# Gyeeta/gyeeta

Hardware: NVIDIA H100
Metric: events/sec aggregated (higher is better)
Workload: dtype u64

## Files before the change

gyeeta_b200/csrc/gysk_tdigest.cuh:

```cuda
#pragma once

#include "gysk_device.cuh"

namespace gysk {

struct TdParams { const double *qtab; uint32_t delta; uint32_t pad; };

template <int NMAX_>
struct TdWorkT
{
	static constexpr int NMAX = NMAX_;
	double			mean[NMAX];
	unsigned long long	pref[NMAX + 1];
	uint16_t		bounds[TD_CAP + 2];
	uint16_t		nxt[NMAX];
	double			src[NMAX];
};
using TdWork = TdWorkT<2 * TD_CAP>;
using TdWorkBig = TdWorkT<1120>;
struct TdScratch : TdWork
{
	Centroid		newc[TD_CAP];
};

template <bool B_STAGED, typename Work>
__device__ __forceinline__ uint32_t td_merge_compress(Work &S, const Centroid *a, uint32_t na, const Centroid *b, uint32_t nb,
		Centroid *out, const TdParams &P)
{
	const int lane = threadIdx.x & 31;
	const uint32_t nm = na + nb;

	double *am = S.src, *bm = S.src + na;
	for (uint32_t j0 = 0; j0 < na; j0 += 32 * 4) {
		double v[4];
#pragma unroll
		for (int q = 0; q < 4; ++q) { const uint32_t j = j0 + q * 32 + lane; v[q] = j < na ? a[j].mean : 0.0; }
#pragma unroll
		for (int q = 0; q < 4; ++q) { const uint32_t j = j0 + q * 32 + lane; if (j < na) am[j] = v[q]; }
	}
	if (!B_STAGED) for (uint32_t j = lane; j < nb; j += 32) bm[j] = b[j].mean;
	__syncwarp();
	const uint32_t per = (nm + 31u) >> 5;
	const uint32_t d0 = lane * per < nm ? lane * per : nm, d1 = d0 + per < nm ? d0 + per : nm;
	unsigned long long tot = 0;
	if (d0 < d1) {
		uint32_t lo = d0 > nb ? d0 - nb : 0u, hi = d0 < na ? d0 : na;
		while (lo < hi) { const uint32_t mid = (lo + hi) >> 1; if (am[mid] <= bm[d0 - 1u - mid]) lo = mid + 1; else hi = mid; }
		uint32_t i = lo, k = d0 - lo;
		double av = i < na ? am[i] : 0.0, bv = k < nb ? bm[k] : 0.0;
		constexpr unsigned long long FROM_A = 1ull << 63;
		for (uint32_t pos = d0; pos < d1; ++pos) {
			const bool ta = i < na && (k >= nb || av <= bv);
			S.mean[pos] = ta ? av : bv;
			if (B_STAGED) S.pref[pos + 1] = ta ? (FROM_A | i) : (unsigned long long)S.nxt[k];
			else S.nxt[pos] = (uint16_t)(ta ? i : (0x8000u | k));
			if (ta) { ++i; av = i < na ? am[i] : 0.0; }
			else { ++k; bv = k < nb ? bm[k] : 0.0; }
		}
		for (uint32_t p0 = d0; p0 < d1; p0 += 4) {
			unsigned long long w[4];
#pragma unroll
			for (int q = 0; q < 4; ++q) {
				const uint32_t pos = p0 + q < d1 ? p0 + q : d1 - 1u;
				if (B_STAGED) { const unsigned long long f = S.pref[pos + 1]; w[q] = (f & FROM_A) ? a[(uint32_t)f].weight : f; }
				else { const uint32_t from = S.nxt[pos]; w[q] = (from & 0x8000u) ? b[from & 0x7FFFu].weight : a[from].weight; }
			}
#pragma unroll
			for (int q = 0; q < 4; ++q) if (p0 + q < d1) { S.pref[p0 + q + 1] = w[q]; tot += w[q]; }
		}
	}
	{
		unsigned long long incl = tot;
#pragma unroll
		for (int off = 1; off < 32; off <<= 1) {
			const unsigned long long tt = __shfl_up_sync(0xffffffffu, incl, off);
			if (lane >= off) incl += tt;
		}
		unsigned long long run = incl - tot;
		for (uint32_t pos = d0; pos < d1; ++pos) { run += S.pref[pos + 1]; S.pref[pos + 1] = run; }
		if (lane == 0) S.pref[0] = 0;
	}
	__syncwarp();
	auto ckey = [&S](uint32_t i) { const unsigned long long p = S.pref[i]; return p + ((S.pref[i + 1] - p) >> 1); };

	uint32_t nout = 0;
	if (nm) {
		const unsigned long long Wt = S.pref[nm];
		const double W = (double)Wt;
		const uint32_t cj = (P.delta + 32u) >> 5;
		uint32_t lo = 0;
		for (uint32_t j = lane * cj, jn = 0; jn < cj && j <= P.delta; ++j, ++jn) {
			const unsigned long long T = j == P.delta ? Wt : (unsigned long long)__dmul_rn(__ldg(P.qtab + j), W);
			uint32_t steps = jn ? 0u : 8u;
			while (steps < 8u && lo < nm && ckey(lo) < T) { ++lo; ++steps; }
			if (steps == 8u) {
				uint32_t hi = nm;
				while (lo < hi) { const uint32_t mid = (lo + hi) >> 1; if (ckey(mid) < T) lo = mid + 1; else hi = mid; }
			}
			S.nxt[j] = (uint16_t)lo;
		}
		__syncwarp();
		for (uint32_t j0 = 0; j0 < P.delta; j0 += 32) {
			const uint32_t j = j0 + lane;
			const bool ne = j < P.delta && S.nxt[j + 1] > S.nxt[j];
			const uint32_t m = __ballot_sync(0xffffffffu, ne);
			if (ne) S.bounds[nout + __popc(m & ((1u << lane) - 1u))] = S.nxt[j];
			nout += __popc(m);
		}
		if (lane == 0) S.bounds[nout] = (uint16_t)nm;
		__syncwarp();
	}

	for (uint32_t c = lane; c < nout; c += 32) {
		double csum = 0.0;
		const uint32_t lo = S.bounds[c], hi = S.bounds[c + 1];
		for (uint32_t i = lo; i < hi; ++i) {
			csum = __dadd_rn(csum, __dmul_rn(S.mean[i], (double)(S.pref[i + 1] - S.pref[i])));
		}
		const unsigned long long cw = S.pref[hi] - S.pref[lo];
		Centroid o; o.mean = __ddiv_rn(csum, (double)cw); o.weight = cw;
		out[c] = o;
	}
	__syncwarp();
	return nout;
}

template <typename Work>
__device__ __forceinline__ uint32_t warp_merge_compress(Work &S, const Centroid *a, uint32_t na, const Centroid *b, uint32_t nb,
		Centroid *out, const TdParams &P)
{
	return td_merge_compress<false>(S, a, na, b, nb, out, P);
}

template <typename Work>
__device__ __forceinline__ uint32_t warp_merge_compress_staged(Work &S, const Centroid *a, uint32_t na, uint32_t nb, Centroid *out,
		const TdParams &P)
{
	return td_merge_compress<true>(S, a, na, nullptr, nb, out, P);
}

}
```

Measured before the change: 13.46 billion.

## Invert t-digest cell lookup per centroid via arcsine estimate and register-cached weights

Instead of binary-searching each of the delta quantile thresholds against the centroid cumulative keys, each merged centroid now estimates its cell index from the arcsine scale function in float and corrects it with a short local walk over a threshold table held in shared scratch. Cell boundaries come from comparing neighbouring cell indices with shuffles and ballots. Input A's weights are also loaded together with the means into registers and staged in shared memory, so the weight gather no longer does scattered global reads. This depends on the float estimate landing close to the right cell, keeps more registers live (sized by TD_CAP), and adds warp syncs.

```diff
diff --git a/gyeeta_b200/csrc/gysk_tdigest.cuh b/gyeeta_b200/csrc/gysk_tdigest.cuh
--- a/gyeeta_b200/csrc/gysk_tdigest.cuh
+++ b/gyeeta_b200/csrc/gysk_tdigest.cuh
@@ -10,6 +10,7 @@
 struct TdWorkT
 {
 	static constexpr int NMAX = NMAX_;
+	static_assert(NMAX > TD_CAP, "the compress keeps the cell starts T_0 .. T_delta (delta <= TD_CAP) in src");
 	double			mean[NMAX];
 	unsigned long long	pref[NMAX + 1];
 	uint16_t		bounds[TD_CAP + 2];
@@ -31,24 +32,28 @@
 	const uint32_t nm = na + nb;
 
 	double *am = S.src, *bm = S.src + na;
-	for (uint32_t j0 = 0; j0 < na; j0 += 32 * 4) {
-		double v[4];
+	unsigned long long aw[TD_CAP / 32];
+	{
+		double v[TD_CAP / 32];
 #pragma unroll
-		for (int q = 0; q < 4; ++q) { const uint32_t j = j0 + q * 32 + lane; v[q] = j < na ? a[j].mean : 0.0; }
+		for (int q = 0; q < TD_CAP / 32; ++q) {
+			const uint32_t j = q * 32 + lane;
+			v[q] = 0.0; aw[q] = 0ull;
+			if (j < na) { const Centroid c = a[j]; v[q] = c.mean; aw[q] = c.weight; }
+		}
 #pragma unroll
-		for (int q = 0; q < 4; ++q) { const uint32_t j = j0 + q * 32 + lane; if (j < na) am[j] = v[q]; }
+		for (int q = 0; q < TD_CAP / 32; ++q) { const uint32_t j = q * 32 + lane; if (j < na) am[j] = v[q]; }
 	}
 	if (!B_STAGED) for (uint32_t j = lane; j < nb; j += 32) bm[j] = b[j].mean;
 	__syncwarp();
 	const uint32_t per = (nm + 31u) >> 5;
 	const uint32_t d0 = lane * per < nm ? lane * per : nm, d1 = d0 + per < nm ? d0 + per : nm;
-	unsigned long long tot = 0;
+	constexpr unsigned long long FROM_A = 1ull << 63;
 	if (d0 < d1) {
 		uint32_t lo = d0 > nb ? d0 - nb : 0u, hi = d0 < na ? d0 : na;
 		while (lo < hi) { const uint32_t mid = (lo + hi) >> 1; if (am[mid] <= bm[d0 - 1u - mid]) lo = mid + 1; else hi = mid; }
 		uint32_t i = lo, k = d0 - lo;
 		double av = i < na ? am[i] : 0.0, bv = k < nb ? bm[k] : 0.0;
-		constexpr unsigned long long FROM_A = 1ull << 63;
 		for (uint32_t pos = d0; pos < d1; ++pos) {
 			const bool ta = i < na && (k >= nb || av <= bv);
 			S.mean[pos] = ta ? av : bv;
@@ -57,17 +62,23 @@
 			if (ta) { ++i; av = i < na ? am[i] : 0.0; }
 			else { ++k; bv = k < nb ? bm[k] : 0.0; }
 		}
-		for (uint32_t p0 = d0; p0 < d1; p0 += 4) {
-			unsigned long long w[4];
+	}
+	__syncwarp();
+	unsigned long long *const aws = reinterpret_cast<unsigned long long *>(S.src);
 #pragma unroll
-			for (int q = 0; q < 4; ++q) {
-				const uint32_t pos = p0 + q < d1 ? p0 + q : d1 - 1u;
-				if (B_STAGED) { const unsigned long long f = S.pref[pos + 1]; w[q] = (f & FROM_A) ? a[(uint32_t)f].weight : f; }
-				else { const uint32_t from = S.nxt[pos]; w[q] = (from & 0x8000u) ? b[from & 0x7FFFu].weight : a[from].weight; }
-			}
+	for (int q = 0; q < TD_CAP / 32; ++q) { const uint32_t j = q * 32 + lane; if (j < na) aws[j] = aw[q]; }
+	__syncwarp();
+	unsigned long long tot = 0;
+	for (uint32_t p0 = d0; p0 < d1; p0 += 4) {
+		unsigned long long w[4];
 #pragma unroll
-			for (int q = 0; q < 4; ++q) if (p0 + q < d1) { S.pref[p0 + q + 1] = w[q]; tot += w[q]; }
+		for (int q = 0; q < 4; ++q) {
+			const uint32_t pos = p0 + q < d1 ? p0 + q : d1 - 1u;
+			if (B_STAGED) { const unsigned long long f = S.pref[pos + 1]; w[q] = (f & FROM_A) ? aws[(uint32_t)f] : f; }
+			else { const uint32_t from = S.nxt[pos]; w[q] = (from & 0x8000u) ? b[from & 0x7FFFu].weight : aws[from]; }
 		}
+#pragma unroll
+		for (int q = 0; q < 4; ++q) if (p0 + q < d1) { S.pref[p0 + q + 1] = w[q]; tot += w[q]; }
 	}
 	{
 		unsigned long long incl = tot;
@@ -81,31 +92,42 @@
 		if (lane == 0) S.pref[0] = 0;
 	}
 	__syncwarp();
-	auto ckey = [&S](uint32_t i) { const unsigned long long p = S.pref[i]; return p + ((S.pref[i + 1] - p) >> 1); };
 
 	uint32_t nout = 0;
 	if (nm) {
 		const unsigned long long Wt = S.pref[nm];
 		const double W = (double)Wt;
-		const uint32_t cj = (P.delta + 32u) >> 5;
-		uint32_t lo = 0;
-		for (uint32_t j = lane * cj, jn = 0; jn < cj && j <= P.delta; ++j, ++jn) {
-			const unsigned long long T = j == P.delta ? Wt : (unsigned long long)__dmul_rn(__ldg(P.qtab + j), W);
-			uint32_t steps = jn ? 0u : 8u;
-			while (steps < 8u && lo < nm && ckey(lo) < T) { ++lo; ++steps; }
-			if (steps == 8u) {
-				uint32_t hi = nm;
-				while (lo < hi) { const uint32_t mid = (lo + hi) >> 1; if (ckey(mid) < T) lo = mid + 1; else hi = mid; }
+		const uint32_t delta = P.delta;
+		unsigned long long *const T = reinterpret_cast<unsigned long long *>(S.src);
+		for (uint32_t j = lane; j <= delta; j += 32) T[j] = j < delta ? (unsigned long long)__dmul_rn(__ldg(P.qtab + j), W) : ~0ull;
+		__syncwarp();
+		const float rw = 1.0f / __ull2float_rn(Wt), kd = (float)delta * 0.318309886f, hd = 0.5f * (float)delta;
+		uint32_t prev = ~0u;
+		for (uint32_t i0 = 0; i0 < nm; i0 += 64) {
+			unsigned long long c[2], t0[2], t1[2];
+			uint32_t j[2];
+#pragma unroll
+			for (int r = 0; r < 2; ++r) {
+				const uint32_t i = i0 + 32u * r + lane;
+				const unsigned long long p = i < nm ? S.pref[i] : 0ull, q = i < nm ? S.pref[i + 1] : 0ull;
+				c[r] = p + ((q - p) >> 1);
+				const float g = fmaf(asinf(fminf(fmaf(2.0f * __ull2float_rn(c[r]), rw, -1.0f), 1.0f)), kd, hd);
+				j[r] = min(__float2uint_rz(g), delta - 1u);
+				t0[r] = T[j[r]]; t1[r] = T[j[r] + 1];
 			}
-			S.nxt[j] = (uint16_t)lo;
-		}
-		__syncwarp();
-		for (uint32_t j0 = 0; j0 < P.delta; j0 += 32) {
-			const uint32_t j = j0 + lane;
-			const bool ne = j < P.delta && S.nxt[j + 1] > S.nxt[j];
-			const uint32_t m = __ballot_sync(0xffffffffu, ne);
-			if (ne) S.bounds[nout + __popc(m & ((1u << lane) - 1u))] = S.nxt[j];
-			nout += __popc(m);
+#pragma unroll
+			for (int r = 0; r < 2; ++r) {
+				uint32_t k = j[r];
+				if (t0[r] > c[r]) { do --k; while (T[k] > c[r]); }
+				else if (t1[r] <= c[r]) { do ++k; while (T[k + 1] <= c[r]); }
+				const uint32_t i = i0 + 32u * r + lane, cl = i < nm ? k : ~0u;
+				const uint32_t up = __shfl_up_sync(0xffffffffu, cl, 1);
+				const bool st = i < nm && cl != (lane ? up : prev);
+				const uint32_t m = __ballot_sync(0xffffffffu, st);
+				if (st) S.bounds[nout + __popc(m & ((1u << lane) - 1u))] = (uint16_t)i;
+				nout += __popc(m);
+				prev = __shfl_sync(0xffffffffu, cl, 31);
+			}
 		}
 		if (lane == 0) S.bounds[nout] = (uint16_t)nm;
 		__syncwarp();
```

Result: no change. 13.61 billion, median of 6 (+1.1%).
